# JJJerome/rl4mm

Hardware: NVIDIA B200
Metric: lob_messages_per_sec (higher is better)
Workload: dtype int32

## Files before the change

rl4mm_b200/csrc/book_flat.cuh:

```cuda
#pragma once
#include "book_fast.cuh"

struct FlatState {
  int n0, n1;
  uint32_t seq;
};

template <class LT>
__host__ __device__ constexpr int flat_nch() { return (LT::NL >= 128 && LT::NO >= 256) ? 4 : 2; }
template <class LT>
__host__ __device__ constexpr int flat_cap() { return 32 * flat_nch<LT>(); }

template <class LT>
__device__ __forceinline__ uint4* flat_pool(unsigned char* blob, int s) {
  static_assert(LT::NO * 8 >= flat_cap<LT>() * 16, "the flat pool (FLAT_CAP x 16 B) lives in the order array of the side");
  static_assert(LT::NO * 8 >= flat_cap<LT>() * 12, "flat_leave: sorted orders (8 B) + one price per order (4 B) in the order array");
  static_assert(LT::NL >= flat_cap<LT>(), "a flat side may hold FLAT_CAP distinct prices");
  static_assert(LT::ord_off % 16 == 0 && LT::side_stride % 16 == 0 && LT::side_off % 16 == 0, "16-byte aligned pool");
  return reinterpret_cast<uint4*>(blob + LT::side_off + s * LT::side_stride + LT::ord_off);
}

template <int NCH>
__device__ __forceinline__ void flat_keys(const uint4* pool, int n, int lane, uint2 (&k)[NCH]) {
#pragma unroll
  for (int c = 0; c < NCH; c++) {
    k[c] = make_uint2(0u, 0xffffffffu);
    if (c * 32 + lane < n) k[c] = *reinterpret_cast<const uint2*>(&pool[c * 32 + lane]);
  }
}
template <int NCH>
__device__ __forceinline__ void flat_keys_raw(const uint4* pool, int lane, uint2 (&k)[NCH]) {
#pragma unroll
  for (int c = 0; c < NCH; c++) k[c] = *reinterpret_cast<const uint2*>(&pool[c * 32 + lane]);
}
template <int NCH>
__device__ __forceinline__ int flat_first(const unsigned (&m)[NCH]) {
  int i = 0;
#pragma unroll
  for (int c = NCH - 1; c >= 0; c--) if (m[c]) i = c * 32 + __ffs(m[c]) - 1;
  return i;
}
template <int S, int NCH>
__device__ __forceinline__ int flat_best_of(const uint2 (&k)[NCH], int n, int lane, int skip) {
  int b = S ? INT32_MAX : INT32_MIN;
#pragma unroll
  for (int c = 0; c < NCH; c++) {
    const int i = c * 32 + lane;
    if (i < n && i != skip) b = S ? min(b, (int)k[c].x) : max(b, (int)k[c].x);
  }
  return S ? __reduce_min_sync(FULL_MASK, b) : __reduce_max_sync(FULL_MASK, b);
}
template <class LT, int S>
__device__ __forceinline__ int flat_best_scan(unsigned char* blob, int lane, int n) {
  uint2 k[flat_nch<LT>()];
  flat_keys(flat_pool<LT>(blob, S), n, lane, k);
  return flat_best_of<S>(k, n, lane, -1);
}

#define FLAT_BAIL_FULL 3
template <class LT, int S, bool TR, bool VCHK = true>
__device__ __forceinline__ bool flat_order(unsigned char* blob, int lane, FastState& f, FlatState& st, int type, int price, int vol, uint32_t ref, bool is_agent) {
  constexpr int OPP = S ^ 1;
  constexpr int NCH = flat_nch<LT>();
  if (!TR) is_agent = false;
  int& n_own = S ? st.n1 : st.n0;
  int& n_opp = S ? st.n0 : st.n1;
  int& best_own = S ? f.best1 : f.best0;
  int& best_opp = S ? f.best0 : f.best1;
  uint4* own = flat_pool<LT>(blob, S);
  uint4* opp = flat_pool<LT>(blob, OPP);
  FastBook<LT> fb; fb.blob = blob; fb.lane = lane;
  if (VCHK && __builtin_expect(vol <= 0, 0)) { f.err |= LOBSIM_ERR_BAD_VOLUME; return false; }
  __syncwarp();
  auto rest = [&](int rem) -> bool {
    if (TR && is_agent) {
      BookHdr* h = reinterpret_cast<BookHdr*>(blob);
      const int nag = h->nag[S];
      if (nag >= LT::NA) { f.err |= LOBSIM_ERR_AGENT_OVERFLOW; return false; }
      const uint32_t id = h->next_agent_id;
      ref = LOBSIM_REF_AGENT | id;
      __syncwarp();
      if (lane == 0) {
        int32_t* ap = reinterpret_cast<int32_t*>(blob + LT::agent_off + S * LT::NA * 12);
        ap[nag] = price; ap[LT::NA + nag] = rem; reinterpret_cast<uint32_t*>(ap)[2 * LT::NA + nag] = id;
        h->nag[S] = nag + 1; h->next_agent_id = id + 1;
      }
    }
    if (lane == 0) own[n_own] = make_uint4((unsigned)price, ref, (unsigned)rem, st.seq);
    n_own += 1; st.seq += 1;
    if (S ? price < best_own : price > best_own) best_own = price;
    return false;
  };
  auto remove = [&]() -> bool {
    uint2 k[NCH];
    flat_keys_raw(own, lane, k);
    int mine = -1;
#pragma unroll
    for (int c = 0; c < NCH; c++) if (c * 32 + lane < n_own && (int)k[c].x == price && k[c].y == ref) mine = c * 32 + lane;
    int i = __reduce_max_sync(FULL_MASK, mine);
    bool aggregate = false;
    if (i < 0) {
      mine = INT32_MAX;
#pragma unroll
      for (int c = NCH - 1; c >= 0; c--) if (c * 32 + lane < n_own && (int)k[c].x == price && k[c].y == LOBSIM_REF_AGGREGATE) mine = c * 32 + lane;
      i = __reduce_min_sync(FULL_MASK, mine);
      if (i == INT32_MAX) return false;
      aggregate = true;
    }
    const int cur = (int)own[i].z;
    __syncwarp();
    if (vol < cur) {
      if (lane == 0) own[i].z = (unsigned)(cur - vol);
      if (TR && is_agent && !aggregate) { __syncwarp(); fast_agent_reduce(fb, S, ref & 0x7fffffffu, vol, false); }
      return false;
    }
    if (price == best_own) best_own = flat_best_of<S>(k, n_own, lane, i);
    if (lane == 0) own[i] = own[n_own - 1];
    n_own -= 1;
    if (TR && is_agent && !aggregate) { __syncwarp(); fast_agent_reduce(fb, S, ref & 0x7fffffffu, cur, true); }
    return false;
  };
  int type2 = type;
  asm volatile("" : "+r"(type2));
  if (__builtin_expect(type == LOBSIM_MSG_LIMIT, 1)) {
    const bool crosses = S ? price <= best_opp : price >= best_opp;
    if (__builtin_expect(!crosses & (n_own < flat_cap<LT>()), 1)) return rest(vol);
    if (n_own >= flat_cap<LT>()) { f.bail = FLAT_BAIL_FULL; return true; }
  } else if (type2 != LOBSIM_MSG_MARKET) return remove();
  {
    int rem = vol;
    {
#pragma unroll 1
      while (rem > 0) {
        if (n_opp == 0) {
          if (type == LOBSIM_MSG_MARKET) { f.err |= LOBSIM_ERR_EMPTY_BOOK; f.dead = 1; return true; }
          break;
        }
        const int bp = best_opp;
        if (type == LOBSIM_MSG_LIMIT && !(S ? price <= bp : price >= bp)) break;
        unsigned q[NCH], qmin = 0xffffffffu;
#pragma unroll
        for (int c = 0; c < NCH; c++) {
          q[c] = 0xffffffffu;
          if (c * 32 + lane < n_opp) { const uint4 e = opp[c * 32 + lane]; if ((int)e.x == bp) q[c] = e.w; }
          qmin = min(qmin, q[c]);
        }
        const unsigned head_seq = __reduce_min_sync(FULL_MASK, qmin);
        int at_best = 0, head = -1;
#pragma unroll
        for (int c = 0; c < NCH; c++) {
          if (q[c] == head_seq) head = c * 32 + lane;
          at_best += __popc(__ballot_sync(FULL_MASK, q[c] != 0xffffffffu));
        }
        const int i = __reduce_max_sync(FULL_MASK, head);
        const uint4 he = opp[i];
        const int hv = (int)he.z;
        const uint32_t href = he.y;
        const bool hagent = TR && (href & LOBSIM_REF_AGENT) != 0;
        const bool self_match = TR && is_agent && hagent;
        if (!self_match) {
          const int v = rem < hv ? rem : hv;
          if (TR) {
            if (hagent) fast_record(fb, f, 0, OPP, bp, v, 0, href);
            else fast_record(fb, f, 1, OPP, bp, v, 0, href);
            if (is_agent) fast_record(fb, f, 0, S, bp, v, 1, href);
          }
          if (rem < hv) {
            __syncwarp();
            if (lane == 0) opp[i].z = (unsigned)(hv - rem);
            if (TR && hagent) { __syncwarp(); fast_agent_reduce(fb, OPP, href & 0x7fffffffu, rem, false); }
            rem = 0;
            break;
          }
          rem -= hv;
        }
        if (at_best == 1) {
          uint2 k[NCH];
          flat_keys(opp, n_opp, lane, k);
          best_opp = flat_best_of<OPP>(k, n_opp, lane, i);
        }
        __syncwarp();
        if (lane == 0) opp[i] = opp[n_opp - 1];
        n_opp -= 1;
        __syncwarp();
        if (TR && hagent) fast_agent_reduce(fb, OPP, href & 0x7fffffffu, 0, true);
      }
    }
    if (!(rem > 0 && type == LOBSIM_MSG_LIMIT)) return false;
    return rest(rem);
  }
  return remove();
}

template <class LT, bool VCHK = true>
__device__ __forceinline__ bool flat_message(unsigned char* blob, int lane, FastState& f, FlatState& st, int price, int vol, uint32_t ref, uint32_t meta) {
  const int type = (int)(meta & 7u);
  if (meta & 8u) return flat_order<LT, 1, false, VCHK>(blob, lane, f, st, type, price, vol, ref, false);
  return flat_order<LT, 0, false, VCHK>(blob, lane, f, st, type, price, vol, ref, false);
}
template <class LT>
__device__ __forceinline__ bool flat_order_tracked(unsigned char* blob, int lane, FastState& f, FlatState& st, int type, int side, int price, int vol, uint32_t ref, bool is_agent) {
  if (side) flat_order<LT, 1, true>(blob, lane, f, st, type, price, vol, ref, is_agent);
  else flat_order<LT, 0, true>(blob, lane, f, st, type, price, vol, ref, is_agent);
  if (f.bail) { f.bail = 0; return false; }
  return true;
}

template <class LT, int S>
__device__ __forceinline__ int flat_best_volume(unsigned char* blob, int lane, const FastState& f, const FlatState& st) {
  const int n = S ? st.n1 : st.n0, best = S ? f.best1 : f.best0;
  const uint4* pool = flat_pool<LT>(blob, S);
  int v = 0;
#pragma unroll
  for (int c = 0; c < flat_nch<LT>(); c++)
    if (c * 32 + lane < n) { const uint4 e = pool[c * 32 + lane]; if ((int)e.x == best) v += (int)e.z; }
  return __reduce_add_sync(FULL_MASK, v);
}

template <class LT>
__device__ __forceinline__ bool flat_fits(const FastBook<LT>& fb, int slack) {
  return fb.cnt(0)->y <= flat_cap<LT>() - slack && fb.cnt(1)->y <= flat_cap<LT>() - slack;
}
template <class LT>
static __device__ __noinline__ int2 flat_enter_fn(unsigned char* blob, int lane) {
  constexpr int NCH = flat_nch<LT>();
  FastBook<LT> fb; fb.blob = blob; fb.lane = lane;
  int2 out = make_int2(0, 0);
  __syncwarp();
#pragma unroll 1
  for (int s = 0; s < 2; s++) {
    unsigned char* sb = fb.side(s);
    const int2 c = *fb.cnt(s);
    const int nlv = c.x, n = c.y;
    uint2 o[NCH]; int pr[NCH];
#pragma unroll
    for (int ch = 0; ch < NCH; ch++) {
      const int i = ch * 32 + lane;
      o[ch] = make_uint2(0u, 0u); pr[ch] = 0;
      if (i < n) {
        o[ch] = fb.O(sb)[i];
        int lo = 0, hi = nlv - 1;
#pragma unroll 1
        while (lo < hi) { const int mid = (lo + hi) >> 1; if ((int)fb.LE(sb)[mid] > i) hi = mid; else lo = mid + 1; }
        pr[ch] = fb.P(sb)[lo];
      }
    }
    __syncwarp();
    uint4* pool = flat_pool<LT>(blob, s);
#pragma unroll
    for (int ch = 0; ch < NCH; ch++) {
      const int i = ch * 32 + lane;
      if (i < n) pool[i] = make_uint4((unsigned)pr[ch], o[ch].y, o[ch].x, (unsigned)i);
    }
    if (s) out.y = n; else out.x = n;
  }
  __syncwarp();
  return out;
}
template <class LT>
__device__ __forceinline__ void flat_enter(const FastBook<LT>& fb, FlatState& st) {
  const int2 n = flat_enter_fn<LT>(fb.blob, fb.lane);
  st.n0 = n.x; st.n1 = n.y; st.seq = (uint32_t)flat_cap<LT>();
}

template <class LT>
static __device__ __noinline__ void flat_leave_fn(unsigned char* blob, int lane, int n0, int n1) {
  constexpr int NCH = flat_nch<LT>();
  FastBook<LT> fb; fb.blob = blob; fb.lane = lane;
  __syncwarp();
#pragma unroll 1
  for (int s = 0; s < 2; s++) {
    unsigned char* sb = fb.side(s);
    const uint4* pool = flat_pool<LT>(blob, s);
    const int n = s ? n1 : n0;
    const unsigned flip = s ? 0xffffffffu : 0u;
    uint4 e[NCH]; unsigned long long k[NCH]; int r[NCH];
#pragma unroll
    for (int c = 0; c < NCH; c++) {
      e[c] = make_uint4(0u, 0u, 0u, 0u);
      if (c * 32 + lane < n) e[c] = pool[c * 32 + lane];
      k[c] = ((unsigned long long)((e[c].x ^ 0x80000000u) ^ flip) << 32) | e[c].w;
      r[c] = 0;
    }
#pragma unroll 1
    for (int m = 0; m < n; m++) {
      const uint4 em = pool[m];
      const unsigned long long km = ((unsigned long long)((em.x ^ 0x80000000u) ^ flip) << 32) | em.w;
#pragma unroll
      for (int c = 0; c < NCH; c++) r[c] += km < k[c] ? 1 : 0;
    }
    __syncwarp();
    int32_t* tmp = reinterpret_cast<int32_t*>(fb.O(sb) + flat_cap<LT>());
#pragma unroll
    for (int c = 0; c < NCH; c++)
      if (c * 32 + lane < n) { fb.O(sb)[r[c]] = make_uint2(e[c].z, e[c].y); tmp[r[c]] = (int)e[c].x; }
    __syncwarp();
    int t[NCH]; unsigned nb[NCH + 1]; int below = 0;
#pragma unroll
    for (int c = 0; c < NCH; c++) {
      const int i = c * 32 + lane;
      t[c] = 0; int pv = 0;
      if (i < n) t[c] = tmp[i];
      if (i > 0 && i < n) pv = tmp[i - 1];
      nb[c] = __ballot_sync(FULL_MASK, i < n && (i == 0 || t[c] != pv));
    }
    nb[NCH] = 0;
    const unsigned le_mask = 0xffffffffu >> (31 - lane);
#pragma unroll
    for (int c = 0; c < NCH; c++) {
      const int i = c * 32 + lane;
      const int lvl = below + __popc(nb[c] & le_mask) - 1;
      const bool is_new = (nb[c] >> lane) & 1u;
      const bool next_new = lane == 31 ? (nb[c + 1] & 1u) != 0 : ((nb[c] >> (lane + 1)) & 1u) != 0;
      if (is_new) fb.P(sb)[lvl] = t[c];
      if (i < n && (i == n - 1 || next_new)) fb.LE(sb)[lvl] = (uint16_t)(i + 1);
      below += __popc(nb[c]);
    }
    if (lane == 0) *fb.cnt(s) = make_int2(below, n);
    __syncwarp();
  }
}
template <class LT>
__device__ __forceinline__ void flat_leave(const FastBook<LT>& fb, const FlatState& st) { flat_leave_fn<LT>(fb.blob, fb.lane, st.n0, st.n1); }

__device__ __forceinline__ bool flat_resync_needed(const BookHdr* h, const int32_t* __restrict__ row, int L, int lane) {
  const int min_buy = h->min_buy, max_sell = h->max_sell;
  unsigned any = 0;
  for (int base = 0; base < 2 * L; base += 32) {
    const int idx = base + lane;
    int price = LOBSIM_NO_PRICE;
    if (idx < 2 * L) price = __ldg(&row[idx * 2]);
    any |= __ballot_sync(FULL_MASK, price != LOBSIM_NO_PRICE && (idx < L ? price < min_buy : price > max_sell));
  }
  return any != 0;
}
template <class LT>
__device__ __forceinline__ void flat_update_trackers(unsigned char* blob, int lane, const FlatState& st) {
  BookHdr* h = reinterpret_cast<BookHdr*>(blob);
  __syncwarp();
  uint2 k[flat_nch<LT>()];
  flat_keys(flat_pool<LT>(blob, 0), st.n0, lane, k);
  const int w0 = flat_best_of<1>(k, st.n0, lane, -1);
  flat_keys(flat_pool<LT>(blob, 1), st.n1, lane, k);
  const int w1 = flat_best_of<0>(k, st.n1, lane, -1);
  if (lane == 0) {
    if (st.n0 && w0 < h->min_buy) h->min_buy = w0;
    if (st.n1 && w1 > h->max_sell) h->max_sell = w1;
  }
  __syncwarp();
}
```

rl4mm_b200/csrc/kernels.cuh:

```cuda
#pragma once
#include <cuda_runtime.h>
#include <stdint.h>

#include <type_traits>
#include "book_flat.cuh"
#include "book_hybrid.cuh"
#include "env.cuh"
#include "lobsim.h"

__device__ __forceinline__ uint32_t smem_u32(const void* p) { return (uint32_t)__cvta_generic_to_shared(p); }
__device__ __forceinline__ void mbar_init(uint64_t* bar, int count) {
  asm volatile("mbarrier.init.shared::cta.b64 [%0], %1;" ::"r"(smem_u32(bar)), "r"(count));
}
__device__ __forceinline__ void fence_mbar_init() { asm volatile("fence.mbarrier_init.release.cluster;" ::: "memory"); }
__device__ __forceinline__ void fence_proxy_async() { asm volatile("fence.proxy.async.shared::cta;" ::: "memory"); }
__device__ __forceinline__ void mbar_expect_tx(uint64_t* bar, uint32_t bytes) {
  asm volatile("mbarrier.arrive.expect_tx.shared::cta.b64 _, [%0], %1;" ::"r"(smem_u32(bar)), "r"(bytes) : "memory");
}
__device__ __forceinline__ bool mbar_try_wait(uint64_t* bar, uint32_t parity) {
  uint32_t ok;
  asm volatile(
      "{\n"
      ".reg .pred p;\n"
      "mbarrier.try_wait.parity.shared::cta.b64 p, [%1], %2;\n"
// ... 395 lines not shown
      const uint4* mp = reinterpret_cast<const uint4*>(msgbuf + (tile & 1) * MSG_TILE_BYTES) + (g % MSG_TILE);
      const unsigned cnt = lim - g;
#pragma unroll 1
      for (unsigned i = 0; i < cnt; i++) {
        const uint4 m = mp[i];
        fast_message(fb, f, (int)m.x, (int)m.y, m.z, m.w);
        if (f.dead) break;
      }
      if (f.dead) break;
      g = lim;
      if (g == tile_end) { __syncwarp(); issue_tile(); }
    }
    if (f.dead) break;
    now_step++;
    if (++sub == steps_per_sec) {
      sub = 0;
      if (c.resync && (!p.resync_last_only || t == T - 1)) {
        const double prop = ec.outer_prop;
        const double bb = f.best0 == INT32_MIN ? 0.0 : (double)f.best0;
        const double bs = f.best1 == INT32_MAX ? (double)INFINITY : (double)f.best1;
        if (bb < (double)h->min_buy + prop * (double)h->init_buy_range || bs > (double)h->max_sell - prop * (double)h->init_sell_range) {
          const int sec = now_step / steps_per_sec;
          if (sec <= (int)stp->n_seconds && stp->snap_valid[sec]) {
            const int32_t* row = stp->snapshots + (size_t)sec * 2 * c.n_levels * 2;
            fast_resync(fb, f, row, c.n_levels);
          }
        }
      }
    }
  }
  while (next_wait < next_issue) wait_tile();
  __syncwarp();
  if (lane == 0) { h->now_step = now_step; h->err = f.err; h->dead = f.dead; }
  __syncwarp();
  fence_proxy_async();
  __syncwarp();
  if (lane == 0) { tma_store(gblob, base, (uint32_t)LT::agent_off); tma_store_wait(); }
  __syncwarp();
}

__device__ __forceinline__ bool hdr_is_flat(const BookHdr* h) { return h->cnt[0][0] < 0; }
template <class LT>
__global__ void __launch_bounds__(128, 3) k_replay_hyb(const __grid_constant__ AdvParams p, const __grid_constant__ EnvConst ec) {
  extern __shared__ __align__(128) unsigned char smem[];
  const int warp = threadIdx.x >> 5, lane = threadIdx.x & 31;
  const int env = blockIdx.x * (blockDim.x >> 5) + warp;
  if (env >= p.n_sel) return;
  const lobsim_cfg_t& c = ec.cfg;
  unsigned char* base = warp_smem_base(smem, warp, p.warp_smem);
  unsigned char* msgbuf = base + LT::agent_off;
  uint64_t* bars = reinterpret_cast<uint64_t*>(msgbuf + 2 * MSG_TILE_BYTES);
  unsigned char* gblob = p.blobs + (size_t)env * LT::blob_bytes;
  if (lane == 0) {
    mbar_init(&bars[0], 1); mbar_init(&bars[1], 1); mbar_init(&bars[2], 1);
    fence_mbar_init();
    mbar_expect_tx(&bars[2], (uint32_t)LT::agent_off);
    tma_load(base, gblob, (uint32_t)LT::agent_off, &bars[2]);
  }
  __syncwarp();
  mbar_wait(&bars[2], 0);

  FastBook<LT> fb; fb.blob = base; fb.lane = lane;
  BookHdr* h = reinterpret_cast<BookHdr*>(base);
  FastState f; f.err = h->err; f.dead = h->dead; f.bail = 0; f.bail_vol = 0;
  if (hdr_is_flat(h)) flat_leave_fn<LT>(base, lane, h->cnt[0][1], h->cnt[1][1]);
  fast_refresh_best(fb, f);
  HybState hs; hs.n0 = hs.n1 = 0; hs.floor0 = INT32_MIN; hs.floor1 = INT32_MAX; hs.seq = 0;
  bool hyb = false;
  const lobsim_stream_t* stp = &p.streams[h->stream_id];
  const lobsim_msg_t* __restrict__ st_msgs = stp->msgs;
  const uint32_t* __restrict__ st_step_off = stp->step_off;
  int now_step = h->now_step;
  const int T = p.T;
  const int n_grid = (int)stp->n_grid_steps;
  if ((now_step < 0 || now_step > n_grid) && !f.dead && T > 0) { f.err |= LOBSIM_ERR_END_OF_STREAM; f.dead = 1; }
  unsigned g = 0, g_end_all = 0;
  if (!f.dead && T > 0) { g = __ldg(&st_step_off[now_step]); g_end_all = __ldg(&st_step_off[min((long long)now_step + T, (long long)n_grid)]); }
  auto try_enter = [&]() {
    if (hyb_enter(fb, f, hs)) hyb = true;
    else if (hs.n0 | hs.n1) { hyb_leave(fb, f, hs); hs.n0 = hs.n1 = 0; }
  };
  if (g < g_end_all) try_enter();
  const unsigned tile0 = g / MSG_TILE;
  unsigned next_issue = 0, next_wait = 0;
  auto issue_tile = [&]() {
    const unsigned first = (tile0 + next_issue) * MSG_TILE;
    if (first >= g_end_all) return;
    if (lane == 0) {
      const unsigned n_total = (unsigned)stp->n_msgs;
      const unsigned cnt = n_total - first < MSG_TILE ? n_total - first : MSG_TILE;
      uint64_t* bar = &bars[next_issue & 1];
      mbar_expect_tx(bar, cnt * 16);
      tma_load(msgbuf + (next_issue & 1) * MSG_TILE_BYTES, st_msgs + first, cnt * 16, bar);
    }
    next_issue++;
  };
  auto wait_tile = [&]() { mbar_wait(&bars[next_wait & 1], (next_wait >> 1) & 1); next_wait++; };
  if (g < g_end_all) { issue_tile(); issue_tile(); }
  __syncwarp();
  const int steps_per_sec = ec.steps_per_sec;
  int sub = now_step >= 0 ? now_step % steps_per_sec : 0;

#pragma unroll 1
  for (int t = 0; t < T && !f.dead; t++) {
    if (now_step >= n_grid) { f.err |= LOBSIM_ERR_END_OF_STREAM; f.dead = 1; break; }
    const unsigned g_step_end = __ldg(&st_step_off[now_step + 1]);
#pragma unroll 1
    while (g < g_step_end) {
      const unsigned tile = g / MSG_TILE - tile0;
      if (tile == next_wait) wait_tile();
      const unsigned tile_end = (g / MSG_TILE + 1) * MSG_TILE;
      const unsigned lim = g_step_end < tile_end ? g_step_end : tile_end;
      const uint4* mp = reinterpret_cast<const uint4*>(msgbuf + (tile & 1) * MSG_TILE_BYTES) + (g % MSG_TILE);
      const unsigned cnt = lim - g;
      unsigned i = 0;
      int redo_vol = 0;
      if (hyb && __any_sync(FULL_MASK, (unsigned)lane < cnt && (int)mp[(unsigned)lane < cnt ? lane : 0].y <= 0)) {
        hyb_leave(fb, f, hs); hyb = false; hs.n0 = hs.n1 = 0;
      }
      if (hyb) {
#pragma unroll 1
        for (; i < cnt; i++) {
          const uint4 m = mp[i];
          if (hyb_message<LT>(fb, f, hs, (int)m.x, (int)m.y, m.z, m.w)) break;
        }
        if (f.bail) {
          const int why = f.bail, rest = f.bail_vol;
          f.bail = 0; f.bail_vol = 0;
          hyb_leave(fb, f, hs); hyb = false; hs.n0 = hs.n1 = 0;
          if (why == FLAT_BAIL_FULL) redo_vol = rest;
          else i++;
        }
      }
      if (!hyb && !f.dead) {
#pragma unroll 1
        for (; i < cnt; i++) {
          const uint4 m = mp[i];
          const int v = redo_vol ? redo_vol : (int)m.y;
          redo_vol = 0;
          fast_message(fb, f, (int)m.x, v, m.z, m.w);
          if (f.dead) break;
        }
      }
      if (f.dead) break;
      g = lim;
      if (g == tile_end) { __syncwarp(); issue_tile(); }
    }
    if (f.dead) break;
    now_step++;
    if (hyb) hyb_top_up(fb, f, hs);
    if (++sub == steps_per_sec) {
      sub = 0;
      if (c.resync && (!p.resync_last_only || t == T - 1)) {
        const double prop = ec.outer_prop;
        const double bb = f.best0 == INT32_MIN ? 0.0 : (double)f.best0;
        const double bs = f.best1 == INT32_MAX ? (double)INFINITY : (double)f.best1;
        if (bb < (double)h->min_buy + prop * (double)h->init_buy_range || bs > (double)h->max_sell - prop * (double)h->init_sell_range) {
          const int sec = now_step / steps_per_sec;
          if (sec <= (int)stp->n_seconds && stp->snap_valid[sec]) {
            const int32_t* row = stp->snapshots + (size_t)sec * 2 * c.n_levels * 2;
            if (hyb && !flat_resync_needed(h, row, c.n_levels, lane)) hyb_update_trackers(fb, hs);
            else {
              if (hyb) { hyb_leave(fb, f, hs); hyb = false; hs.n0 = hs.n1 = 0; }
              fast_resync(fb, f, row, c.n_levels);
            }
          }
        }
      }
      if (!hyb) try_enter();
    }
  }
  if (hyb) hyb_leave(fb, f, hs);
  while (next_wait < next_issue) wait_tile();
  __syncwarp();
  if (lane == 0) { h->now_step = now_step; h->err = f.err; h->dead = f.dead; }
  __syncwarp();
  fence_proxy_async();
  __syncwarp();
  if (lane == 0) { tma_store(gblob, base, (uint32_t)LT::agent_off); tma_store_wait(); }
  __syncwarp();
}

template <class LT, bool LOAD>
__device__ __forceinline__ uint32_t flat_body_copy(unsigned char* sm, unsigned char* gm, uint64_t* bar, int lane, int n0, int n1) {
  const BookHdr* h = reinterpret_cast<const BookHdr*>(sm);
  uint32_t off = 0, len = 0;
  if (lane < 2) { off = LT::side_off + lane * LT::side_stride + LT::ord_off; len = (uint32_t)(lane ? n1 : n0) * 16u; }
  else if (lane < 8) {
    const int s = (lane - 2) / 3, part = (lane - 2) % 3;
    off = LT::agent_off + s * LT::NA * 12 + part * LT::NA * 4;
    len = (min((uint32_t)h->nag[s], (uint32_t)LT::NA) * 4 + 15) & ~15u;
  }
  const uint32_t total = __reduce_add_sync(FULL_MASK, len);
  if (total == 0) return 0;
  if (LOAD) { if (lane == 0) mbar_expect_tx(bar, total); __syncwarp(); }
  if (len) { if (LOAD) tma_load(sm + off, gm + off, len, bar); else tma_store_part(gm + off, sm + off, len); }
  return total;
}
template <class LT>
__device__ __forceinline__ void flat_adopt(unsigned char* sm, int lane, FastState& f, FlatState& fs) {
  const BookHdr* h = reinterpret_cast<const BookHdr*>(sm);
  fs.n0 = h->cnt[0][1]; fs.n1 = h->cnt[1][1]; fs.seq = (uint32_t)h->cnt[1][0];
  f.best0 = flat_best_scan<LT, 0>(sm, lane, fs.n0);
  f.best1 = flat_best_scan<LT, 1>(sm, lane, fs.n1);
}
__device__ __forceinline__ void flat_mark(BookHdr* h, const FlatState& fs) {
  h->cnt[0][0] = -1; h->cnt[0][1] = fs.n0; h->cnt[1][0] = (int32_t)fs.seq; h->cnt[1][1] = fs.n1;
}

template <class LT>
__global__ void __launch_bounds__(128) k_to_sorted(unsigned char* blobs, int n_envs) {
  extern __shared__ __align__(128) unsigned char smem[];
  const int warp = threadIdx.x >> 5, lane = threadIdx.x & 31;
  const int env = blockIdx.x * (blockDim.x >> 5) + warp;
  if (env >= n_envs) return;
  unsigned char* gblob = blobs + (size_t)env * LT::blob_bytes;
  if (!hdr_is_flat(reinterpret_cast<const BookHdr*>(gblob))) return;
  unsigned char* base = smem + (size_t)warp * LT::blob_bytes;
  if (lane < 8) reinterpret_cast<uint4*>(base)[lane] = reinterpret_cast<const uint4*>(gblob)[lane];
  __syncwarp();
  const BookHdr* h = reinterpret_cast<const BookHdr*>(base);
  FlatState fs; fs.n0 = h->cnt[0][1]; fs.n1 = h->cnt[1][1]; fs.seq = (uint32_t)h->cnt[1][0];
#pragma unroll
  for (int s = 0; s < 2; s++) {
    const int n = s ? fs.n1 : fs.n0;
    const uint4* gp = flat_pool<LT>(gblob, s); uint4* sp = flat_pool<LT>(base, s);
    for (int i = lane; i < n; i += 32) sp[i] = gp[i];
  }
  __syncwarp();
  FastBook<LT> fb; fb.blob = base; fb.lane = lane;
  flat_leave(fb, fs);
  __syncwarp();
  if (lane == 0) reinterpret_cast<uint4*>(gblob)[0] = reinterpret_cast<const uint4*>(base)[0];
#pragma unroll
  for (int s = 0; s < 2; s++) {
    const int2 c = *fb.cnt(s);
    unsigned char* ss = fb.side(s); unsigned char* gs = gblob + LT::side_off + s * LT::side_stride;
    for (int i = lane; i < c.x; i += 32) { fb.P(gs)[i] = fb.P(ss)[i]; fb.LE(gs)[i] = fb.LE(ss)[i]; }
    for (int i = lane; i < c.y; i += 32) fb.O(gs)[i] = fb.O(ss)[i];
  }
}

#ifndef LOBSIM_REPLAY_FLAT_MIN_BLOCKS
#define LOBSIM_REPLAY_FLAT_MIN_BLOCKS 7
#endif
template <class LT>
__global__ void __launch_bounds__(128, LOBSIM_REPLAY_FLAT_MIN_BLOCKS) k_replay_flat(const __grid_constant__ AdvParams p, const __grid_constant__ EnvConst ec) {
  extern __shared__ __align__(128) unsigned char smem[];
  const int warp = threadIdx.x >> 5, lane = threadIdx.x & 31;
  const int env = blockIdx.x * (blockDim.x >> 5) + warp;
  if (env >= p.n_sel) return;
  const lobsim_cfg_t& c = ec.cfg;
  unsigned char* base = warp_smem_base(smem, warp, p.warp_smem);
  unsigned char* msgbuf = base + LT::agent_off;
  uint64_t* bars = reinterpret_cast<uint64_t*>(msgbuf + 2 * MSG_TILE_BYTES);
  unsigned char* gblob = p.blobs + (size_t)env * LT::blob_bytes;
  if (lane == 0) {
    mbar_init(&bars[0], 1); mbar_init(&bars[1], 1); mbar_init(&bars[2], 1);
    fence_mbar_init();
    mbar_expect_tx(&bars[2], (uint32_t)LT::agent_off);
    tma_load(base, gblob, (uint32_t)LT::agent_off, &bars[2]);
  }
  __syncwarp();
  mbar_wait(&bars[2], 0);

  FastBook<LT> fb; fb.blob = base; fb.lane = lane;
  BookHdr* h = reinterpret_cast<BookHdr*>(base);
  FastState f; f.err = h->err; f.dead = h->dead; f.bail = 0; f.bail_vol = 0;
  if (!hdr_is_flat(h)) fast_refresh_best(fb, f);
  FlatState fs; fs.n0 = fs.n1 = 0; fs.seq = 0;
  bool flat = false;
  if (hdr_is_flat(h)) { flat_adopt<LT>(base, lane, f, fs); flat = true; }
  const lobsim_stream_t* stp = &p.streams[h->stream_id];
  const lobsim_msg_t* __restrict__ st_msgs = stp->msgs;
  const uint32_t* __restrict__ st_step_off = stp->step_off;
  int now_step = h->now_step;
  const int T = p.T;
  const int n_grid = (int)stp->n_grid_steps;
  if ((now_step < 0 || now_step > n_grid) && !f.dead && T > 0) { f.err |= LOBSIM_ERR_END_OF_STREAM; f.dead = 1; }
  unsigned g = 0, g_end_all = 0;
  if (!f.dead && T > 0) { g = __ldg(&st_step_off[now_step]); g_end_all = __ldg(&st_step_off[min((long long)now_step + T, (long long)n_grid)]); }
  if (!flat && g < g_end_all && flat_fits(fb, 0)) { flat_enter(fb, fs); flat = true; }
  const unsigned tile0 = g / MSG_TILE;
  unsigned next_issue = 0, next_wait = 0;
  auto issue_tile = [&]() {
    const unsigned first = (tile0 + next_issue) * MSG_TILE;
    if (first >= g_end_all) return;
    if (lane == 0) {
      const unsigned n_total = (unsigned)stp->n_msgs;
      const unsigned cnt = n_total - first < MSG_TILE ? n_total - first : MSG_TILE;
      uint64_t* bar = &bars[next_issue & 1];
      mbar_expect_tx(bar, cnt * 16);
      tma_load(msgbuf + (next_issue & 1) * MSG_TILE_BYTES, st_msgs + first, cnt * 16, bar);
    }
    next_issue++;
  };
  auto wait_tile = [&]() { mbar_wait(&bars[next_wait & 1], (next_wait >> 1) & 1); next_wait++; };
  if (g < g_end_all) { issue_tile(); issue_tile(); }
  __syncwarp();
  const int steps_per_sec = ec.steps_per_sec;
  int sub = now_step >= 0 ? now_step % steps_per_sec : 0;

#pragma unroll 1
  for (int t = 0; t < T && !f.dead; t++) {
    if (now_step >= n_grid) { f.err |= LOBSIM_ERR_END_OF_STREAM; f.dead = 1; break; }
    const unsigned g_step_end = __ldg(&st_step_off[now_step + 1]);
#pragma unroll 1
    while (g < g_step_end) {
      const unsigned tile = g / MSG_TILE - tile0;
      if (tile == next_wait) wait_tile();
      const unsigned tile_end = (g / MSG_TILE + 1) * MSG_TILE;
      const unsigned lim = g_step_end < tile_end ? g_step_end : tile_end;
      const uint4* mp = reinterpret_cast<const uint4*>(msgbuf + (tile & 1) * MSG_TILE_BYTES) + (g % MSG_TILE);
      const unsigned cnt = lim - g;
      unsigned i = 0;
      if (flat) {
        const bool bad_vol = __any_sync(FULL_MASK, (unsigned)lane < cnt && (int)mp[(unsigned)lane < cnt ? lane : 0].y <= 0);
        unsigned off = 0;
        const unsigned off_end = cnt * 16u;
        auto run = [&](auto vchk) {
#pragma unroll 1
          for (; off != off_end; off += 16u) {
            const uint4 m = *reinterpret_cast<const uint4*>(reinterpret_cast<const unsigned char*>(mp) + off);
            if (flat_message<LT, decltype(vchk)::value>(base, lane, f, fs, (int)m.x, (int)m.y, m.z, m.w)) return true;
          }
          return false;
        };
        const bool stopped = __builtin_expect(bad_vol, 0) ? run(std::true_type{}) : run(std::false_type{});
        i = off >> 4;
        f.bail = 0;
        if (stopped && !f.dead) { flat_leave(fb, fs); flat = false; }
      }
      if (!flat && !f.dead) {
#pragma unroll 1
        for (; i < cnt; i++) {
          const uint4 m = mp[i];
          fast_message(fb, f, (int)m.x, (int)m.y, m.z, m.w);
          if (f.dead) break;
        }
      }
      if (f.dead) break;
      g = lim;
      if (g == tile_end) { __syncwarp(); issue_tile(); }
    }
    if (f.dead) break;
    now_step++;
    if (++sub == steps_per_sec) {
      sub = 0;
      if (c.resync && (!p.resync_last_only || t == T - 1)) {
        const double prop = ec.outer_prop;
        const double bb = f.best0 == INT32_MIN ? 0.0 : (double)f.best0;
        const double bs = f.best1 == INT32_MAX ? (double)INFINITY : (double)f.best1;
        if (bb < (double)h->min_buy + prop * (double)h->init_buy_range || bs > (double)h->max_sell - prop * (double)h->init_sell_range) {
          const int sec = now_step / steps_per_sec;
          if (sec <= (int)stp->n_seconds && stp->snap_valid[sec]) {
            const int32_t* row = stp->snapshots + (size_t)sec * 2 * c.n_levels * 2;
            if (flat && !flat_resync_needed(h, row, c.n_levels, lane)) flat_update_trackers<LT>(base, lane, fs);
            else {
              if (flat) { flat_leave(fb, fs); flat = false; }
              fast_resync(fb, f, row, c.n_levels);
            }
          }
        }
      }
      if (flat && fs.seq > 0xE0000000u) { flat_leave(fb, fs); flat = false; }
      if (!flat && flat_fits(fb, 8)) { flat_enter(fb, fs); flat = true; }
    }
  }
  if (flat && !p.allow_flat) { flat_leave(fb, fs); flat = false; }
  while (next_wait < next_issue) wait_tile();
  __syncwarp();
  if (lane == 0) { h->now_step = now_step; h->err = f.err; h->dead = f.dead; if (flat) flat_mark(h, fs); }
  __syncwarp();
  fence_proxy_async();
  __syncwarp();
  if (lane == 0) { tma_store(gblob, base, (uint32_t)LT::agent_off); tma_store_wait(); }
  __syncwarp();
}

static __device__ __noinline__ uint32_t reset_book_cold(unsigned char* blob, const Layout* L, int lane, const lobsim_cfg_t* c, const lobsim_stream_t* st, int stream_id, int start_step) {
  Book b; b.blob = blob; b.L = *L; b.lane = lane;
  WarpState w;
  __syncwarp();
  load_state<true>(b, w);
  w.fill_log = nullptr; w.fill_cap = 0; w.n_fills = 0;
  init_book_from_snapshot(b, w, *c, *st, stream_id, start_step);
  store_state<true>(b, w);
  return pack_errdead(w.err, w.dead);
}

template <class LT, bool LOAD>
__device__ __forceinline__ uint32_t blob_body_copy(unsigned char* sm, unsigned char* gm, uint64_t* bar, int lane) {
  static_assert(LT::NL % 8 == 0 && LT::NO % 2 == 0 && LT::NA % 4 == 0 && LT::ord_off % 16 == 0 && LT::side_stride % 16 == 0 && LT::agent_off % 16 == 0,
                "StaticLayout arrays must be 16-byte aligned for the partial blob copies");
  const BookHdr* h = reinterpret_cast<const BookHdr*>(sm);
  const int s = lane >= 6 ? 1 : 0, part = lane - s * 6;
  uint32_t off = 0, len = 0;
  if (lane < 12) {
    const uint32_t so = LT::side_off + s * LT::side_stride, ao = LT::agent_off + s * LT::NA * 12;
    if (part == 0)      { off = so;                 len = min((uint32_t)h->cnt[s][0], (uint32_t)LT::NL) * 4; }
    else if (part == 1) { off = so + LT::lvend_off; len = min((uint32_t)h->cnt[s][0], (uint32_t)LT::NL) * 2; }
    else if (part == 2) { off = so + LT::ord_off;   len = min((uint32_t)h->cnt[s][1], (uint32_t)LT::NO) * 8; }
    else                { off = ao + (part - 3) * LT::NA * 4; len = min((uint32_t)h->nag[s], (uint32_t)LT::NA) * 4; }
    len = (len + 15) & ~15u;
  }
  const uint32_t total = __reduce_add_sync(FULL_MASK, len);
  if (total == 0) return 0;
  if (LOAD) { if (lane == 0) mbar_expect_tx(bar, total); __syncwarp(); }
  if (len) { if (LOAD) tma_load(sm + off, gm + off, len, bar); else tma_store_part(gm + off, sm + off, len); }
  return total;
}

#ifndef LOBSIM_ENVFAST_WARPS
#define LOBSIM_ENVFAST_WARPS 8
#endif
#ifndef LOBSIM_ENVFAST_MINB
#define LOBSIM_ENVFAST_MINB (24 / LOBSIM_ENVFAST_WARPS)
#endif
template <class LT>
constexpr int env_min_blocks() {
  const int warp_bytes = (LT::blob_bytes + 2 * MSG_TILE_BYTES + scratch_bytes(LT::NA) + 32 + 128 + 127) & ~127;
  const int fit = (227 * 1024) / (LOBSIM_ENVFAST_WARPS * warp_bytes);
  return fit < 1 ? 1 : (fit < LOBSIM_ENVFAST_MINB ? fit : LOBSIM_ENVFAST_MINB);
}
#ifndef LOBSIM_PHASE_SYNC
#define LOBSIM_PHASE_SYNC 1
#endif
#define ENV_CLASSIC 0
#define ENV_HOT 1
#define ENV_DEFERRED 2
#ifndef LOBSIM_SYNC_B
#define LOBSIM_SYNC_B 1
#endif
#ifndef LOBSIM_SYNC_C
#define LOBSIM_SYNC_C 1
#endif
#if LOBSIM_PHASE_SYNC
#define PHASE_SYNC() __syncthreads()
#else
#define PHASE_SYNC() ((void)0)
#endif
struct StepSave { double cash0, p0, price; long long inv0, episode_start_us, st_t0_us; };
template <class LT, bool SYNC, bool RARE, int MODE>
__global__ void __launch_bounds__(32 * LOBSIM_ENVFAST_WARPS, env_min_blocks<LT>()) k_env_fast(const __grid_constant__ AdvParams p, const __grid_constant__ EnvConst ec) {
  extern __shared__ __align__(128) unsigned char smem[];
  const int warp = threadIdx.x >> 5, lane = threadIdx.x & 31;
  int sel = p.sel_offset + blockIdx.x * (blockDim.x >> 5) + warp, t_start = 0;
  if (MODE == ENV_DEFERRED) {
    static_assert(MODE != ENV_DEFERRED || !SYNC, "the deferred launch has no block-level barriers");
    if (sel >= *p.defer_count) return;
    const int2 item = p.defer_list[sel];
    sel = item.x; t_start = item.y;
  }
  if (sel >= p.n_sel) return;
  const int env = p.env_ids ? p.env_ids[sel] : sel;
  const lobsim_cfg_t& c = ec.cfg;
  unsigned char* base = warp_smem_base(smem, warp, p.warp_smem);
  unsigned char* msgbuf = base + LT::blob_bytes;
  int2* scratch = reinterpret_cast<int2*>(msgbuf + 2 * MSG_TILE_BYTES);
  uint64_t* bars = reinterpret_cast<uint64_t*>(reinterpret_cast<unsigned char*>(scratch) + scratch_bytes(LT::NA));
  unsigned char* gblob = p.blobs + (size_t)env * LT::blob_bytes;
  if (lane == 0) {
    mbar_init(&bars[0], 1); mbar_init(&bars[1], 1); mbar_init(&bars[2], 1);
    fence_mbar_init();
    mbar_expect_tx(&bars[2], (uint32_t)sizeof(BookHdr));
    tma_load(base, gblob, (uint32_t)sizeof(BookHdr), &bars[2]);
  }
  __syncwarp();
  mbar_wait(&bars[2], 0);
  FastBook<LT> fb; fb.blob = base; fb.lane = lane;
  Book b; b.blob = base; b.L = p.L; b.lane = lane;
  BookHdr* h = reinterpret_cast<BookHdr*>(base);
  bool flat = false;
  bool aborted = false;
  FlatState fs; fs.n0 = fs.n1 = 0; fs.seq = 0;
  auto defer = [&](int t) { aborted = true; if (lane == 0) { const int k = atomicAdd(p.defer_count, 1); p.defer_list[k] = make_int2(sel, t); } };
  if (!p.reset_mode) {
    if (hdr_is_flat(h)) {
      if (flat_body_copy<LT, true>(base, gblob, &bars[2], lane, h->cnt[0][1], h->cnt[1][1])) mbar_wait(&bars[2], 1);
      if (MODE == ENV_HOT) flat = true;
      else flat_leave_fn<LT>(base, lane, h->cnt[0][1], h->cnt[1][1]);
    } else if (blob_body_copy<LT, true>(base, gblob, &bars[2], lane)) mbar_wait(&bars[2], 1);
  }
  FastState f; f.err = h->err; f.dead = h->dead; f.bail = 0; f.bail_vol = 0;
  f.fill_log = p.fill_log ? p.fill_log + (size_t)env * p.fill_cap : nullptr; f.fill_cap = p.fill_cap;
  if (lane == 0) h->n_fills = 0;
  const int F = c.n_features;

  int stream_id = h->stream_id;
  if (p.reset_mode) {
    stream_id = p.reset_stream_ids[sel];
    int start = p.reset_steps[sel] - (p.reset_mode == 2 ? c.warmup_steps : 0);
    if (stream_id < 0 || stream_id >= p.n_streams) { stream_id = 0; start = -1; }
    const uint32_t ed = reset_book_cold(base, &p.L, lane, &ec.cfg, &p.streams[stream_id], stream_id, start);
    f.err = ed & 0x7fffffffu; f.dead = (int)(ed >> 31);
    if (p.reset_mode == 2 && lane == 0) {
      h->episode_start_step = p.reset_steps[sel];
      if (!c.portfolio_carryover || !h->has_reset) { h->inventory = c.initial_inventory; h->cash = c.initial_cash; }
      h->has_reset = 1;
    }
    __syncwarp();
  }
  if (MODE == ENV_HOT && flat) flat_adopt<LT>(base, lane, f, fs);
  else {
    fast_refresh_best(fb, f);
    if (MODE == ENV_HOT) {
      if (flat_fits(fb, 8)) { flat_enter(fb, fs); flat = true; }
      else defer(0);
    }
  }
  const lobsim_stream_t* stp = &p.streams[stream_id];
  const lobsim_msg_t* __restrict__ st_msgs = stp->msgs;
  const uint32_t* __restrict__ st_step_off = stp->step_off;
  StepSave* sv = reinterpret_cast<StepSave*>(bars + 4);
  int now_step = h->now_step;
  if (lane == 0) { sv->st_t0_us = stp->t0_us; sv->episode_start_us = stp->t0_us + (long long)h->episode_start_step * c.step_us; sv->price = h->price; }
  __syncwarp();
  FeatState* fstate_env = p.fstate + (size_t)env * LOBSIM_MAX_FEATURES;
  NormState* nstate_env = RARE && p.nstate ? p.nstate + (size_t)env * LOBSIM_MAX_FEATURES : nullptr;
  double* rings_env = p.rings + (size_t)env * ec.ring_stride;
  double feat_cur = 0.0;
  if (lane < F) feat_cur = fstate_env[lane].cur;
  const int t0_mod_min = (int)stp->reserved;

  auto tops = [&](StepView& v) {
    v.have_tops = f.best0 != INT32_MIN && f.best1 != INT32_MAX;
    if (v.have_tops) {
      v.bb = f.best0; v.bs = f.best1;
      __syncwarp();
      if (MODE == ENV_HOT) { v.bv = flat_best_volume<LT, 0>(base, lane, f, fs); v.sv = flat_best_volume<LT, 1>(base, lane, f, fs); }
      else { v.bv = best_level_volume(b, 0, h->cnt[0][0]); v.sv = best_level_volume(b, 1, h->cnt[1][0]); }
      double imb; v.price = microprice(v.bb, v.bs, v.bv, v.sv, imb);
    } else { v.bb = v.bs = v.bv = v.sv = 0; v.price = NAN; }
  };
  if (p.reset_mode == 2) {
    StepView v; tops(v);
    v.inventory = h->inventory; v.now_us = sv->st_t0_us + (long long)now_step * c.step_us;
    v.us_in_min = us_in_minute(t0_mod_min, now_step, ec);
    v.n_ext0 = v.n_ext1 = v.vol_ext0 = v.vol_ext1 = v.n_int0 = v.n_int1 = v.vol_int0 = v.vol_int1 = 0;
    __syncwarp();
    if (lane == 0) sv->price = v.price;
    feat_cur = features_step<RARE>(&ec, fstate_env, nstate_env, rings_env, lane, v, sv->episode_start_us, 1);
    __syncwarp();
  }

  const int T = p.T;
  const int n_grid = (int)stp->n_grid_steps;
  if ((now_step < 0 || now_step > n_grid) && !f.dead && T > t_start) { f.err |= LOBSIM_ERR_END_OF_STREAM; f.dead = 1; }
  unsigned g = 0, g_end_all = 0;
  if (!f.dead && !aborted && T > t_start) { g = __ldg(&st_step_off[now_step]); g_end_all = __ldg(&st_step_off[min((long long)now_step + (T - t_start), (long long)n_grid)]); }
  const unsigned tile0 = g / MSG_TILE;
  unsigned next_issue = 0, next_wait = 0;
  auto issue_tile = [&]() {
    const unsigned first = (tile0 + next_issue) * MSG_TILE;
    if (first >= g_end_all) return;
    if (lane == 0) {
      const unsigned n_total = (unsigned)stp->n_msgs;
      const unsigned cnt = n_total - first < MSG_TILE ? n_total - first : MSG_TILE;
      uint64_t* bar = &bars[next_issue & 1];
      mbar_expect_tx(bar, cnt * 16);
      tma_load(msgbuf + (next_issue & 1) * MSG_TILE_BYTES, st_msgs + first, cnt * 16, bar);
    }
    next_issue++;
  };
  auto wait_tile = [&]() { mbar_wait(&bars[next_wait & 1], (next_wait >> 1) & 1); next_wait++; };
  if (g < g_end_all) { issue_tile(); issue_tile(); }
  __syncwarp();
  if (SYNC) PHASE_SYNC();
  const int steps_per_sec = ec.steps_per_sec;
  int sub = now_step >= 0 ? now_step % steps_per_sec : 0;

  auto store_blob = [&]() {
    __syncwarp();
    if (lane == 0) {
      if (f.fill_log && h->n_fills > f.fill_cap) f.err |= LOBSIM_ERR_FILL_LOG_FULL;
      h->now_step = now_step; h->price = sv->price; h->err = f.err; h->dead = f.dead;
      if (p.fill_count) p.fill_count[env] = h->n_fills;
      if (MODE == ENV_HOT) flat_mark(h, fs);
    }
    __syncwarp();
    fence_proxy_async();
    __syncwarp();
    if (lane == 12) tma_store_part(gblob, base, (uint32_t)sizeof(BookHdr));
    if (MODE == ENV_HOT) flat_body_copy<LT, false>(base, gblob, nullptr, lane, fs.n0, fs.n1);
    else blob_body_copy<LT, false>(base, gblob, nullptr, lane);
    if (lane <= 12) { tma_store_commit(); tma_store_wait(); }
    __syncwarp();
  };
  AgentGenFast gen; gen.side = 3; gen.stage = 0; gen.need = 0; gen.todo0 = gen.todo1 = gen.wm0 = gen.wm1 = 0; gen.wide_removed = gen.wide_pos = 0;
  gen.pending_id = 0; gen.base0 = gen.base1 = 0; gen.clear_vol = -1; gen.clear_side = 0;
  const int Q = c.max_quote_level - c.min_quote_level;
  int* diff_scratch = reinterpret_cast<int*>(scratch);
  bool agent_phase = false;
#pragma unroll 1
  for (int t = t_start; t < T; t++) {
    if (SYNC) PHASE_SYNC();
    __syncwarp();
    if (lane == 0) { sv->cash0 = h->cash; sv->p0 = sv->price; sv->inv0 = h->inventory; }
    if (lane < 8) h->flow[lane] = 0;
    __syncwarp();
    if (p.agent_kind != LOBSIM_AGENT_NONE && !(MODE == ENV_HOT && aborted)) {
      double* act_sm = reinterpret_cast<double*>(scratch);
      if (p.agent_kind == LOBSIM_AGENT_EXTERNAL) {
        const double* a = p.actions_in + ((size_t)t * p.n_sel + sel) * ec.action_dim;
        if (lane < 5) act_sm[lane] = lane < ec.action_dim ? __ldg(&a[lane]) : 0.0;
      } else {
        const lobsim_agent_t* agp = p.agents ? p.agents + sel : &p.agent;
        const double inv_obs = __shfl_sync(FULL_MASK, feat_cur, agp->inventory_index & 31);
        if (lane == 0) agent_action_cold(agp, inv_obs, act_sm, env, now_step);
      }
      __syncwarp();
      const double a0 = act_sm[0], a1 = act_sm[1], a2 = act_sm[2], a3 = act_sm[3], a4 = act_sm[4];
      const double mine = lane < 5 ? act_sm[lane] : 0.0;
      __syncwarp();
      if (p.act && p.agent_kind != LOBSIM_AGENT_EXTERNAL && lane < ec.action_dim) p.act[((size_t)t * p.n_sel + sel) * ec.action_dim + lane] = mine;
      if (p.obs && !p.out_final_obs_only && c.inc_prev_action_in_obs && lane < ec.action_dim)
        p.obs[((size_t)t * p.n_sel + sel) * ec.obs_dim + F + lane] = mine;
      if (!f.dead) {
        const AgentGen g0 = agent_prepare(b, f.best0, f.best1, h->nag[0], h->nag[1], h->inventory, &ec, a0, a1, a2, a3, a4, p.beta_tab, diff_scratch);
        f.err |= g0.err_out; if (g0.dead_out) f.dead = 1;
        gen = agent_gen_fast_init(g0, lane, diff_scratch);
        agent_phase = true;
      }
    }
    if (SYNC && LOBSIM_SYNC_B) PHASE_SYNC();
    {
      if (!f.dead && now_step >= (int)stp->n_grid_steps) { f.err |= LOBSIM_ERR_END_OF_STREAM; f.dead = 1; }
      const unsigned g_step_end = f.dead ? g : __ldg(&st_step_off[now_step + 1]);
#pragma unroll 1
      for (;;) {
        int type, side, oprice, vol; uint32_t ref; bool is_agent;
        if (MODE == ENV_HOT && aborted) break;
        if (agent_phase) {
          if (!agent_next_fast(fb, f, gen, diff_scratch, Q, c.tick_size, type, side, oprice, vol, ref)) { agent_phase = false; continue; }
          is_agent = true;
        } else {
          if (f.dead || g >= g_step_end) break;
          const unsigned tile = g / MSG_TILE - tile0;
          if (tile == next_wait) wait_tile();
          const uint4 m = *reinterpret_cast<const uint4*>(msgbuf + (tile & 1) * MSG_TILE_BYTES + (g % MSG_TILE) * 16);
          oprice = (int)m.x; vol = (int)m.y; ref = m.z; type = (int)(m.w & 7u); side = (int)((m.w >> 3) & 1u);
          is_agent = false;
          g++;
          if (g % MSG_TILE == 0) { __syncwarp(); issue_tile(); }
        }
        if (!f.dead) {
          if (MODE == ENV_HOT) { if (!flat_order_tracked<LT>(base, lane, f, fs, type, side, oprice, vol, ref, is_agent)) defer(t); }
          else fast_order_full<LT, true>(fb, f, type, side, oprice, vol, ref, is_agent);
        }
      }
    }
    if (!f.dead && !(MODE == ENV_HOT && aborted)) {
// ... 59 lines not shown
```

Before: 15.24 billion.

## Drop warp syncs in untracked flat path and batch steps per second

```diff
diff --git a/rl4mm_b200/csrc/book_flat.cuh b/rl4mm_b200/csrc/book_flat.cuh
--- a/rl4mm_b200/csrc/book_flat.cuh
+++ b/rl4mm_b200/csrc/book_flat.cuh
@@ -71,7 +71,8 @@
   uint4* opp = flat_pool<LT>(blob, OPP);
   FastBook<LT> fb; fb.blob = blob; fb.lane = lane;
   if (VCHK && __builtin_expect(vol <= 0, 0)) { f.err |= LOBSIM_ERR_BAD_VOLUME; return false; }
-  __syncwarp();
+  const bool wr = !TR || lane == 0;
+  if (TR) __syncwarp();
   auto rest = [&](int rem) -> bool {
     if (TR && is_agent) {
       BookHdr* h = reinterpret_cast<BookHdr*>(blob);
@@ -86,7 +87,7 @@
         h->nag[S] = nag + 1; h->next_agent_id = id + 1;
       }
     }
-    if (lane == 0) own[n_own] = make_uint4((unsigned)price, ref, (unsigned)rem, st.seq);
+    if (wr) own[n_own] = make_uint4((unsigned)price, ref, (unsigned)rem, st.seq);
     n_own += 1; st.seq += 1;
     if (S ? price < best_own : price > best_own) best_own = price;
     return false;
@@ -108,14 +109,14 @@
       aggregate = true;
     }
     const int cur = (int)own[i].z;
-    __syncwarp();
+    if (TR) __syncwarp();
     if (vol < cur) {
-      if (lane == 0) own[i].z = (unsigned)(cur - vol);
+      if (wr) own[i].z = (unsigned)(cur - vol);
       if (TR && is_agent && !aggregate) { __syncwarp(); fast_agent_reduce(fb, S, ref & 0x7fffffffu, vol, false); }
       return false;
     }
     if (price == best_own) best_own = flat_best_of<S>(k, n_own, lane, i);
-    if (lane == 0) own[i] = own[n_own - 1];
+    if (wr) own[i] = own[n_own - 1];
     n_own -= 1;
     if (TR && is_agent && !aggregate) { __syncwarp(); fast_agent_reduce(fb, S, ref & 0x7fffffffu, cur, true); }
     return false;
@@ -166,8 +167,8 @@
             if (is_agent) fast_record(fb, f, 0, S, bp, v, 1, href);
           }
           if (rem < hv) {
-            __syncwarp();
-            if (lane == 0) opp[i].z = (unsigned)(hv - rem);
+            if (TR) __syncwarp();
+            if (wr) opp[i].z = (unsigned)(hv - rem);
             if (TR && hagent) { __syncwarp(); fast_agent_reduce(fb, OPP, href & 0x7fffffffu, rem, false); }
             rem = 0;
             break;
@@ -179,10 +180,10 @@
           flat_keys(opp, n_opp, lane, k);
           best_opp = flat_best_of<OPP>(k, n_opp, lane, i);
         }
-        __syncwarp();
-        if (lane == 0) opp[i] = opp[n_opp - 1];
+        if (TR) __syncwarp();
+        if (wr) opp[i] = opp[n_opp - 1];
         n_opp -= 1;
-        __syncwarp();
+        if (TR) __syncwarp();
         if (TR && hagent) fast_agent_reduce(fb, OPP, href & 0x7fffffffu, 0, true);
       }
     }
diff --git a/rl4mm_b200/csrc/kernels.cuh b/rl4mm_b200/csrc/kernels.cuh
--- a/rl4mm_b200/csrc/kernels.cuh
+++ b/rl4mm_b200/csrc/kernels.cuh
@@ -721,15 +721,16 @@
   int sub = now_step >= 0 ? now_step % steps_per_sec : 0;
 
 #pragma unroll 1
-  for (int t = 0; t < T && !f.dead; t++) {
-    if (now_step >= n_grid) { f.err |= LOBSIM_ERR_END_OF_STREAM; f.dead = 1; break; }
-    const unsigned g_step_end = __ldg(&st_step_off[now_step + 1]);
-#pragma unroll 1
-    while (g < g_step_end) {
+  for (int t = 0; t < T && !f.dead;) {
+    const int k = min(min(steps_per_sec - sub, T - t), n_grid - now_step);
+    if (k <= 0) { f.err |= LOBSIM_ERR_END_OF_STREAM; f.dead = 1; break; }
+    const unsigned g_pass_end = __ldg(&st_step_off[now_step + k]);
+#pragma unroll 1
+    while (g < g_pass_end) {
       const unsigned tile = g / MSG_TILE - tile0;
       if (tile == next_wait) wait_tile();
       const unsigned tile_end = (g / MSG_TILE + 1) * MSG_TILE;
-      const unsigned lim = g_step_end < tile_end ? g_step_end : tile_end;
+      const unsigned lim = g_pass_end < tile_end ? g_pass_end : tile_end;
       const uint4* mp = reinterpret_cast<const uint4*>(msgbuf + (tile & 1) * MSG_TILE_BYTES) + (g % MSG_TILE);
       const unsigned cnt = lim - g;
       unsigned i = 0;
@@ -758,15 +759,18 @@
           if (f.dead) break;
         }
       }
-      if (f.dead) break;
+      if (f.dead) { g += i; break; }
       g = lim;
       if (g == tile_end) { __syncwarp(); issue_tile(); }
     }
-    if (f.dead) break;
-    now_step++;
-    if (++sub == steps_per_sec) {
+    if (f.dead) {
+      while (__ldg(&st_step_off[now_step + 1]) <= g) now_step++;
+      break;
+    }
+    now_step += k; t += k; sub += k;
+    if (sub == steps_per_sec) {
       sub = 0;
-      if (c.resync && (!p.resync_last_only || t == T - 1)) {
+      if (c.resync && (!p.resync_last_only || t == T)) {
         const double prop = ec.outer_prop;
         const double bb = f.best0 == INT32_MIN ? 0.0 : (double)f.best0;
         const double bs = f.best1 == INT32_MAX ? (double)INFINITY : (double)f.best1;
```

New measurement: 17.13 billion (median of 6 runs). 12.4% higher.
